# zachramsey/pm-rl

Measured on AMD Instinct MI355X. Metric: env-steps/sec (whole node) at 65k envs x 30 assets; reward MAE vs CPU ref, higher is better.
Workload: dtype f64

## Files before the change

pm-rl_amd/csrc/step_relay.h:

```cpp
#pragma once
#include "env_step.h"
#include "scalar_vec.h"

namespace pmenv_dev {

struct RelayParams {
    uint32_t scal;
    uint32_t epoch;
    uint64_t* w;
    uint64_t* list;
    uint32_t* done;
    uint32_t spin;
    uint32_t rot;
    uint32_t grid;
    const int32_t* kp_in;
    int32_t* kp_out;
    const float* halo_in;
    float* halo_out;
    uint32_t* seq;
    int32_t* kp;
    float* halo;
    uint32_t B;
    uint32_t halo_stride;
    const float* obs;
    uint32_t par;
};
enum { kSeqD = 0, kSeqE = 1, kSeqV = 2, kSeqC = 3, kSeqEC = 4, kSeqHobs = 6 };

struct RelayCtx {
    uint32_t epoch;
    const int32_t* kp_in;
    int32_t* kp_out;
    const float* halo_in;
    float* halo_out;
};
template <bool SEQ>
__device__ __forceinline__ RelayCtx relay_ctx(const RelayParams& r) {
    RelayCtx c{r.epoch, r.kp_in, r.kp_out, r.halo_in, r.halo_out};
    if constexpr (SEQ) {
        const uint32_t par = __builtin_amdgcn_readfirstlane(r.seq[kSeqC]);
        c.epoch = __builtin_amdgcn_readfirstlane(r.seq[kSeqEC]);
        c.kp_in = r.kp + (size_t)par * r.B;
        c.kp_out = r.kp + (size_t)(par ^ 1u) * r.B;
        c.halo_in = r.halo + (size_t)par * r.halo_stride;
        c.halo_out = r.halo + (size_t)(par ^ 1u) * r.halo_stride;
    }
    return c;
}

struct KArgs {
    StepParams p;
    RelayParams r;
    uint32_t qtot;
};
__device__ __forceinline__ KArgs kargs() {
    typedef __attribute__((address_space(4))) const uint32_t KWord;
    KWord* ka = (KWord*)__builtin_amdgcn_kernarg_segment_ptr();
    asm volatile("" : "+s"(ka));
    uint32_t w[sizeof(KArgs) / 4];
#pragma unroll
    for (size_t i = 0; i < sizeof(KArgs) / 4; ++i) w[i] = ka[i];
    KArgs k;
    __builtin_memcpy(&k, w, sizeof(KArgs));
    return k;
}

constexpr uint32_t kStampSlots = 16, kStampMaxWg = 40960;
static __device__ uint64_t* g_relay_stamps;
template <bool ST, bool DRAIN = false>
__device__ __forceinline__ uint64_t relay_clock(uint32_t dep) {
    uint64_t t = 0;
    if constexpr (ST) {
        if constexpr (DRAIN)
            asm volatile("s_waitcnt vmcnt(0)\n\ts_memrealtime %0\n\ts_waitcnt lgkmcnt(0)" : "=s"(t) : "v"(dep) : "memory");
        else
            asm volatile("s_memrealtime %0\n\ts_waitcnt lgkmcnt(0)" : "=s"(t) : "v"(dep) : "memory");
    }
    return t;
}
template <bool ST, int K>
__device__ __forceinline__ void relay_stamps_put(uint32_t bid, uint32_t epoch, const uint64_t (&ts)[K]) {
    if constexpr (ST) {
        uint64_t* s = g_relay_stamps;
        if (s && threadIdx.x == 0 && bid < kStampMaxWg) {
#pragma unroll
            for (int k = 0; k < K; ++k) s[((size_t)(epoch % kStampSlots) * kStampMaxWg + bid) * 8 + k] = ts[k];
        }
    }
}

__device__ __forceinline__ void relay_put(uint64_t* w, uint32_t epoch, uint32_t bits) {
    __hip_atomic_store(w, ((uint64_t)epoch << 32) | bits, __ATOMIC_RELAXED, __HIP_MEMORY_SCOPE_AGENT);
}
__device__ __forceinline__ uint64_t relay_get(const uint64_t* w) {
    return __hip_atomic_load(const_cast<uint64_t*>(w), __ATOMIC_RELAXED, __HIP_MEMORY_SCOPE_AGENT);
}

__device__ __forceinline__ uint32_t relay_list_read(const RelayParams& r, uint32_t epoch) {
    __atomic_signal_fence(__ATOMIC_SEQ_CST);
    __builtin_amdgcn_s_waitcnt(0);
    __atomic_signal_fence(__ATOMIC_SEQ_CST);
    const uint64_t lw = relay_get(r.list);
    return (uint32_t)(lw >> 32) == epoch ? (uint32_t)lw : 0u;
}

template <int BLOCK, int KL, int KA, bool ST = false>
__device__ __forceinline__ uint32_t relay_scalar(const StepParams& p, const RelayParams& r, int s, uint32_t epoch,
                                                 int32_t* kp_out, uint64_t t_entry = 0) {
    uint64_t ts[3] = {t_entry, 0, 0};
    constexpr int EPW = 64 / KL, EPB = (BLOCK / 64) * EPW;
    const int lane = threadIdx.x & 63;
    const int b = s * EPB + (int)(threadIdx.x >> 6) * EPW + lane / KL;
    const int j = lane % KL;
    const int N = p.N;
    const bool env_ok = b < p.B;
    uint32_t listed;
    if constexpr (KA == 0) {
        const ScalarIn in = scalar_load<KL>(p, b, lane);
        const ScalarMid m = scalar_core<KL>(p, b, lane, in);
        if (env_ok && j < N) relay_put(r.w + (size_t)b * N + j, epoch, __float_as_uint(m.wp));
        if (env_ok && j == 0) kp_out[b] = m.k + 1;
        listed = relay_list_read(r, epoch);
        ts[1] = relay_clock<ST>(listed);
        scalar_tail<KL>(p, b, lane, in, m);
    } else {
        const VecIn<KA> in = vec_load<KL, KA, true>(p, b, lane);
        const VecMid<KA> m = vec_core<KL, KA, true>(p, b, lane, in);
#pragma unroll
        for (int e = 0; e < KA; ++e) {
            const int n = j + e * KL;
            if (env_ok && n < N) relay_put(r.w + (size_t)b * N + n, epoch, __float_as_uint(m.wp[e]));
        }
        if (env_ok && j == 0) kp_out[b] = in.k + 1;
        listed = relay_list_read(r, epoch);
        ts[1] = relay_clock<ST>(listed);
        vec_tail<KL, KA, true>(p, b, lane, in, m);
    }
    ts[2] = relay_clock<ST, true>(0);
    relay_stamps_put<ST>((uint32_t)s, epoch, ts);
    return listed;
}

template <int BLOCK, int V, int POL, bool OUT, bool ADOPT, bool ST = false>
__device__ __forceinline__ bool relay_tile(const StepParams& p, const RelayParams& r, uint32_t qtot, uint32_t spin, uint32_t t,
                                           uint32_t epoch, const int32_t* kp_in, const float* halo_in,
                                           float* halo_out, f4* sh4, f4* sh_bar, float* sh_wp, int32_t* sh_kc,
                                           int32_t* sh_ok, uint64_t t_entry = 0) {
    uint64_t ts[6] = {t_entry, 0, 0, 0, 0, 0};
    constexpr int kAux = POL == 1 ? 2 : 0;
    constexpr int CPW = BLOCK * V, F = 5;
    const int tid = threadIdx.x, lane = tid & 63, wave = tid >> 6;
    const uint32_t c0 = t * CPW;
    const uint32_t nblk = min((uint32_t)CPW, qtot - c0);
    const auto rs = make_rsrc(p.obs + (size_t)c0 * 4, nblk * 16u);
    f4 own[V];
#pragma unroll
    for (int v = 0; v < V; ++v) own[v] = buf_load4<kAux>(rs, (uint32_t)(64 * V * wave + 64 * v + lane) * 16u);
    const uint32_t ntiles = (qtot + CPW - 1) / CPW;
    const uint32_t nh = t + 1 < ntiles ? min(2u, qtot - c0 - nblk) : 0u;
    const float* hsrc = OUT ? p.obs + (size_t)(c0 + nblk) * 4 : halo_in + (size_t)t * 8;
    const f4 hal = buf_load4<0>(make_rsrc(hsrc, nh * 16u), tid < 2 ? (uint32_t)tid * 16u : 0xFFFFFFF0u);
    __builtin_amdgcn_sched_barrier(0);
    const int N = p.N, W = p.W, WF = W * F;
    const uint32_t per4 = (uint32_t)(N * WF) >> 2;
    const uint32_t b_lo = fdiv(c0, p.div_units);
    const uint32_t g_lo = b_lo * (uint32_t)N + fdiv(4u * (c0 - b_lo * per4), p.div_wf);
    const uint32_t ql = c0 + nblk - 1u;
    const uint32_t b_hi = fdiv(ql, p.div_units);
    const uint32_t g_hi = b_hi * (uint32_t)N + fdiv(4u * (ql - b_hi * per4) + 3u, p.div_wf);
    const bool mine = (uint32_t)tid <= g_hi - g_lo;
    const uint32_t g = g_lo + (mine ? (uint32_t)tid : 0u);
    const uint32_t b = g / (uint32_t)N, n = g - b * (uint32_t)N;
    const float* barb = env_bar(p, (int)b);
    const float nanv = __int_as_float(0x7fc00000);
    f4 xb = f4{nanv, nanv, nanv, nanv};
    int32_t kc = 0;
    uint64_t ww = 0;
    if (barb) xb = *reinterpret_cast<const f4*>(barb + (size_t)n * 4);
    kc = kp_in[b];
    ww = relay_get(r.w + g);
    bool ready = !mine || (uint32_t)(ww >> 32) == epoch;
    ts[1] = relay_clock<ST>((uint32_t)ww);
    for (uint32_t polls = 0; !ADOPT && !__all(ready) && polls < spin; ++polls) {
        __builtin_amdgcn_s_sleep(2);
        if (!ready) {
            ww = relay_get(r.w + g);
            ready = (uint32_t)(ww >> 32) == epoch;
        }
    }
    const bool wave_ok = __all(ready);
    ts[2] = relay_clock<ST>((uint32_t)ww);
    if (mine) {
        sh_bar[tid] = xb;
        sh_wp[tid] = __uint_as_float((uint32_t)ww);
        sh_kc[tid] = kc;
    }
#pragma unroll
    for (int v = 0; v < V; ++v) sh4[64 * V * wave + 64 * v + lane] = own[v];
    if (tid < 2) sh4[CPW + tid] = hal;
    if (lane == 0) sh_ok[wave] = wave_ok ? 1 : 0;
    __syncthreads();
    ts[3] = relay_clock<ST>(0);
    if constexpr (ADOPT) {
        bool tile_ok = true;
#pragma unroll
        for (int w = 0; w < BLOCK / 64; ++w) tile_ok = tile_ok && sh_ok[w] != 0;
        if (!tile_ok) return false;
        if (tid == 0)
            sh_ok[BLOCK / 64] = __hip_atomic_exchange(r.done + t, epoch, __ATOMIC_RELAXED, __HIP_MEMORY_SCOPE_AGENT) != epoch;
        __syncthreads();
        if (!sh_ok[BLOCK / 64]) return true;
    }
    const auto rd = OUT ? make_rsrc(p.obs_out + (size_t)c0 * 4, nblk * 16u) : rs;
    const bool first_out = !OUT && t > 0;
    bool ok = true;
#pragma unroll
    for (int v = 0; v < V; ++v) {
        const int j = 64 * V * wave + 64 * v + lane;
        const uint32_t q = min(c0 + (uint32_t)j, qtot - 1u);
        const uint32_t bq = fdiv(q, p.div_units);
        const uint32_t j0 = 4u * (q - bq * per4);
        const uint32_t row = fdiv(j0, p.div_wf);
        const int kk = (int)(j0 - row * (uint32_t)WF);
        const int i = (int)(bq * (uint32_t)N + row - g_lo);
        const f4 n1 = sh4[j + 1], n2 = sh4[j + 2];
        const float sh[4] = {n1.y, n1.z, n1.w, n2.x};
        const float un[4] = {own[v].x, own[v].y, own[v].z, own[v].w};
        f4 o = compose2(p, kk, sh_kc[i], un, sh, [&](f4& x, float& xwp) {
            x = sh_bar[i];
            xwp = sh_wp[i];
        });
        if (!ADOPT && v == 0) {
            int32_t okv = 1;
#pragma unroll
            for (int w = 0; w < BLOCK / 64; ++w) okv &= sh_ok[w];
            ok = __builtin_amdgcn_readfirstlane(okv) != 0;
        }
        buf_store4<kAux>(rd, ok ? (uint32_t)j * 16u : 0x80000000u, o);
        if (ok && first_out && j < 2) reinterpret_cast<f4*>(halo_out)[2 * (t - 1) + j] = o;
    }
    ts[4] = relay_clock<ST>(0);
    ts[5] = relay_clock<ST, true>(0);
    relay_stamps_put<ST>(r.scal + t, epoch, ts);
    return ok;
}

template <int BLOCK, int V, int POL, bool OUT, bool SEQ>
__device__ __forceinline__ void relay_adopt(f4* sh4, f4* sh_bar, float* sh_wp, int32_t* sh_kc, int32_t* sh_ok,
                                            uint32_t listed) {
    constexpr int kB = BLOCK / 64 + 1;
    const int wave = threadIdx.x >> 6;
    if ((threadIdx.x & 63) == 0) sh_ok[wave] = (int32_t)__builtin_amdgcn_readfirstlane(listed);
    __syncthreads();
    uint32_t n = 0;
#pragma unroll
    for (int w = 0; w < BLOCK / 64; ++w) n = max(n, (uint32_t)sh_ok[w]);
    if (n == 0) return;
    const KArgs ka = kargs();
    const RelayCtx c = relay_ctx<SEQ>(ka.r);
    for (uint32_t i = 0; i < n; ++i) {
        __syncthreads();
        if (threadIdx.x == 0) {
            const uint64_t e = relay_get(ka.r.list + 1 + i);
            int32_t t = (uint32_t)(e >> 32) == c.epoch ? (int32_t)(uint32_t)e : -1;
            if (t >= 0 && __hip_atomic_load(ka.r.done + t, __ATOMIC_RELAXED, __HIP_MEMORY_SCOPE_AGENT) == c.epoch)
                t = -1;
            sh_ok[kB] = t;
        }
        __syncthreads();
        const int32_t t = __builtin_amdgcn_readfirstlane(sh_ok[kB]);
        if (t >= 0)
            (void)relay_tile<BLOCK, V, POL, OUT, true>(ka.p, ka.r, ka.qtot, 0u, (uint32_t)t, c.epoch, c.kp_in, c.halo_in,
                                                       c.halo_out, sh4, sh_bar, sh_wp, sh_kc, sh_ok);
    }
}

template <int BLOCK, int V, int POL, bool OUT, bool SEQ>
__device__ __forceinline__ void relay_defer(uint32_t t, f4* sh4, f4* sh_bar, float* sh_wp, int32_t* sh_kc,
                                            int32_t* sh_ok) {
    const KArgs ka = kargs();
    const RelayCtx c = relay_ctx<SEQ>(ka.r);
    if (threadIdx.x == 0) {
        uint64_t lw = relay_get(ka.r.list), nw;
        do {
            nw = (uint32_t)(lw >> 32) == c.epoch ? lw + 1 : ((uint64_t)c.epoch << 32) | 1u;
        } while (!__hip_atomic_compare_exchange_strong(ka.r.list, &lw, nw, __ATOMIC_RELAXED, __ATOMIC_RELAXED,
                                                        __HIP_MEMORY_SCOPE_AGENT));
        const uint32_t slot = (uint32_t)(lw >> 32) == c.epoch ? (uint32_t)lw : 0u;
        relay_put(ka.r.list + 1 + slot, c.epoch, t);
        __atomic_signal_fence(__ATOMIC_SEQ_CST);
        __builtin_amdgcn_s_waitcnt(0);
        __atomic_signal_fence(__ATOMIC_SEQ_CST);
    }
    __syncthreads();
    (void)relay_tile<BLOCK, V, POL, OUT, true>(ka.p, ka.r, ka.qtot, 0u, t, c.epoch, c.kp_in, c.halo_in, c.halo_out, sh4,
                                               sh_bar, sh_wp, sh_kc, sh_ok);
}

template <int BLOCK, int V, int POL, bool OUT, int KL, int KA, int OCC = 1, bool SEQ = false, int ANY = 0>
__global__ __launch_bounds__(BLOCK) __attribute__((amdgpu_waves_per_eu(OCC))) void step_relay_kernel(
    StepParams p, RelayParams r, uint32_t qtot) {
    __shared__ f4 sh4[BLOCK * V + 2];
    __shared__ f4 sh_bar[BLOCK];
    __shared__ float sh_wp[BLOCK];
    __shared__ int32_t sh_kc[BLOCK];
    __shared__ int32_t sh_ok[BLOCK / 64 + 2];
    const RelayCtx c = relay_ctx<SEQ>(r);
    if constexpr (SEQ) {
        if (blockIdx.x == 0 && threadIdx.x == 0) {
            const uint64_t hobs = OUT ? 0ull : (uint64_t)(uintptr_t)r.obs;
            r.seq[kSeqD] = (uint32_t)((c.kp_in - r.kp) / r.B) ^ 1u;
            r.seq[kSeqE] = c.epoch;
            r.seq[kSeqV] = 1u;
            r.seq[kSeqHobs] = (uint32_t)hobs;
            r.seq[kSeqHobs + 1] = (uint32_t)(hobs >> 32);
        }
    }
    constexpr bool kSt = ANY == 2;
    const uint64_t t_entry = relay_clock<kSt>(0);
    uint32_t bid = blockIdx.x;
    if constexpr (ANY == 1) {
        bid += r.rot;
        if (bid >= r.grid) bid -= r.grid;
    }
    if (bid < r.scal) {
        const uint32_t listed = relay_scalar<BLOCK, KL, KA, kSt>(p, r, (int)bid, c.epoch, c.kp_out, t_entry);
        relay_adopt<BLOCK, V, POL, OUT, SEQ>(sh4, sh_bar, sh_wp, sh_kc, sh_ok, listed);
    } else if (!relay_tile<BLOCK, V, POL, OUT, false, kSt>(p, r, qtot, ANY == 1 ? r.spin : kRelaySpin, bid - r.scal, c.epoch,
                                                           c.kp_in, c.halo_in, c.halo_out, sh4, sh_bar, sh_wp, sh_kc,
                                                           sh_ok, t_entry)) {
        relay_defer<BLOCK, V, POL, OUT, SEQ>(bid - r.scal, sh4, sh_bar, sh_wp, sh_kc, sh_ok);
    }
}

static __global__ __launch_bounds__(256) void relay_prime_kernel(StepParams p, RelayParams r, int prime_kp, int seq) {
    uint32_t d = r.par;
    bool kp = prime_kp != 0, halo = p.halo != nullptr;
    if (seq) {
        d = __builtin_amdgcn_readfirstlane(r.seq[kSeqD]);
        const uint32_t e = __builtin_amdgcn_readfirstlane(r.seq[kSeqE]);
        const uint32_t v = __builtin_amdgcn_readfirstlane(r.seq[kSeqV]);
        const uint64_t hobs = (uint64_t)__builtin_amdgcn_readfirstlane(r.seq[kSeqHobs]) |
                              ((uint64_t)__builtin_amdgcn_readfirstlane(r.seq[kSeqHobs + 1]) << 32);
        kp = v == 0;
        halo = halo && (v == 0 || hobs != (uint64_t)(uintptr_t)p.obs);
        if (blockIdx.x == 0 && threadIdx.x == 0) {
            r.seq[kSeqC] = d;
            r.seq[kSeqEC] = e + 1u == 0u ? 1u : e + 1u;
        }
    }
    if (halo) {
        p.halo += (size_t)d * r.halo_stride;
        copy_halo(p);
    }
    if (kp) {
        int32_t* kpd = r.kp + (size_t)d * r.B;
        for (int b = blockIdx.x * blockDim.x + threadIdx.x; b < p.B; b += gridDim.x * blockDim.x) kpd[b] = p.k[b];
    }
}

}
```

Measured before the change: 103.8 million.

## Patch new bar rows into shared image and shift uniformly in relay compose

Adds a tile-wide vote that records whether every row shifts or every row is a full-storage ring. When the tile is uniform, each owning thread writes its new bar and weight directly into the shared observation image, and the output becomes a plain four-float shift, with weight slots optionally taken from the unshifted data. This replaces the per-element index divisions and compose2 branching with simple shared-memory reads. Mixed tiles fall back to the old compose path, now with unroll disabled. The cost is an extra barrier-phase patch step and more code paths that must stay bit-exact.

Result: no change. 103.8 million (-0.0%).

```diff
diff --git a/pm-rl_amd/csrc/relay_patch.h b/pm-rl_amd/csrc/relay_patch.h
--- /dev/null
+++ b/pm-rl_amd/csrc/relay_patch.h
@@ -0,0 +1,61 @@
+#pragma once
+
+#include <stdint.h>
+
+#if defined(__HIPCC__)
+#define PMENV_HD __host__ __device__ __forceinline__
+#else
+#define PMENV_HD inline
+#endif
+
+namespace pmenv_dev {
+
+constexpr int kRelayF = 5;
+constexpr int kRelayHaloFloats = 8;
+
+enum { kVoteOk = 1, kVoteShift = 2, kVoteFull = 4 };
+
+PMENV_HD int relay_image_floats(int cpw) { return 4 * cpw + kRelayHaloFloats; }
+
+PMENV_HD bool relay_row_shifts(bool storage_ring, int32_t k, int W) { return !(storage_ring && k >= W - 1); }
+
+PMENV_HD int32_t relay_vote(bool wave_ok, bool any_shift, bool any_full) {
+    return (wave_ok ? kVoteOk : 0) | (any_shift ? kVoteShift : 0) | (any_full ? kVoteFull : 0);
+}
+PMENV_HD int32_t relay_vote_fold(int32_t all_and, int32_t all_or) {
+    return (all_and & kVoteOk) | (all_or & (kVoteShift | kVoteFull));
+}
+PMENV_HD bool relay_vote_ok(int32_t tile_vote) { return (tile_vote & kVoteOk) != 0; }
+PMENV_HD bool relay_vote_plain(int32_t tile_vote) {
+    return (tile_vote & (kVoteShift | kVoteFull)) != (kVoteShift | kVoteFull);
+}
+PMENV_HD bool relay_vote_full(int32_t tile_vote) { return (tile_vote & (kVoteShift | kVoteFull)) == kVoteFull; }
+
+PMENV_HD int relay_base0(uint32_t chunk_in_env, uint32_t row_lo, int WF) {
+    return (int)(row_lo * (uint32_t)WF) - (int)(4u * chunk_in_env);
+}
+
+PMENV_HD bool relay_in_image(int pos, int image_floats) { return (uint32_t)pos < (uint32_t)image_floats; }
+
+template <typename Put>
+PMENV_HD void relay_patch_row(int i, int base0, int WF, int image_floats, bool shifts, int slot, Put put) {
+    const int row_end = base0 + (i + 1) * WF;
+    if (relay_in_image(row_end, image_floats)) put(row_end, 0);
+    if (relay_in_image(row_end + 1, image_floats)) put(row_end + 1, 1);
+    if (relay_in_image(row_end + 2, image_floats)) put(row_end + 2, 2);
+    if (relay_in_image(row_end + 3, image_floats)) put(row_end + 3, 3);
+    const int wpos = shifts ? row_end + (kRelayF - 1) : row_end - WF + kRelayF * slot + (kRelayF - 1);
+    if (relay_in_image(wpos, image_floats)) put(wpos, kRelayF - 1);
+}
+
+PMENV_HD int relay_f0(uint32_t q) {
+    const uint32_t r = q % (uint32_t)kRelayF;
+    return r ? kRelayF - (int)r : 0;
+}
+PMENV_HD int relay_f0_step(int f0, int steps) {
+    const int f = f0 + steps % kRelayF;
+    return f >= kRelayF ? f - kRelayF : f;
+}
+PMENV_HD bool relay_is_weight(int f0, int e) { return f0 + e == kRelayF - 1 || f0 + e == 2 * kRelayF - 1; }
+
+}
diff --git a/pm-rl_amd/csrc/step_relay.h b/pm-rl_amd/csrc/step_relay.h
--- a/pm-rl_amd/csrc/step_relay.h
+++ b/pm-rl_amd/csrc/step_relay.h
@@ -1,5 +1,8 @@
 #pragma once
+#include <type_traits>
+
 #include "env_step.h"
+#include "relay_patch.h"
 #include "scalar_vec.h"
 
 namespace pmenv_dev {
@@ -190,54 +193,91 @@
     }
     const bool wave_ok = __all(ready);
     ts[2] = relay_clock<ST>((uint32_t)ww);
+    const bool shifts = relay_row_shifts(p.ring_mode == PMENV_RING_STORAGE, kc, W);
+    const int32_t wave_vote = relay_vote(wave_ok, __any(mine && shifts) != 0, __any(mine && !shifts) != 0);
+    const float wp = __uint_as_float((uint32_t)ww);
     if (mine) {
         sh_bar[tid] = xb;
-        sh_wp[tid] = __uint_as_float((uint32_t)ww);
+        sh_wp[tid] = wp;
         sh_kc[tid] = kc;
     }
 #pragma unroll
     for (int v = 0; v < V; ++v) sh4[64 * V * wave + 64 * v + lane] = own[v];
     if (tid < 2) sh4[CPW + tid] = hal;
-    if (lane == 0) sh_ok[wave] = wave_ok ? 1 : 0;
+    if (lane == 0) sh_ok[wave] = wave_vote;
+    __syncthreads();
+    int32_t v_and = kVoteOk, v_or = 0;
+#pragma unroll
+    for (int w = 0; w < BLOCK / 64; ++w) {
+        const int32_t x = sh_ok[w];
+        v_and &= x;
+        v_or |= x;
+    }
+    const int32_t vote = __builtin_amdgcn_readfirstlane(relay_vote_fold(v_and, v_or));
+    if constexpr (ADOPT) {
+        if (!relay_vote_ok(vote)) return false;
+        if (tid == 0)
+            sh_ok[BLOCK / 64] = __hip_atomic_exchange(r.done + t, epoch, __ATOMIC_RELAXED, __HIP_MEMORY_SCOPE_AGENT) != epoch;
+    }
+    const bool plain = relay_vote_plain(vote), full = relay_vote_full(vote);
+    if (plain && mine) {
+        const uint32_t cq = c0 - b_lo * per4;
+        const int slot = (int)((uint32_t)(1 + kc) - fdiv((uint32_t)(1 + kc), p.div_w) * (uint32_t)W);
+        float* img = reinterpret_cast<float*>(sh4);
+        relay_patch_row(tid, relay_base0(cq, g_lo - b_lo * (uint32_t)N, WF), WF, relay_image_floats(CPW), shifts, slot,
+                        [&](int pos, int c) { img[pos] = c == 0 ? xb.x : c == 1 ? xb.y : c == 2 ? xb.z : c == 3 ? xb.w : wp; });
+    }
     __syncthreads();
     ts[3] = relay_clock<ST>(0);
     if constexpr (ADOPT) {
-        bool tile_ok = true;
-#pragma unroll
-        for (int w = 0; w < BLOCK / 64; ++w) tile_ok = tile_ok && sh_ok[w] != 0;
-        if (!tile_ok) return false;
-        if (tid == 0)
-            sh_ok[BLOCK / 64] = __hip_atomic_exchange(r.done + t, epoch, __ATOMIC_RELAXED, __HIP_MEMORY_SCOPE_AGENT) != epoch;
-        __syncthreads();
         if (!sh_ok[BLOCK / 64]) return true;
     }
     const auto rd = OUT ? make_rsrc(p.obs_out + (size_t)c0 * 4, nblk * 16u) : rs;
     const bool first_out = !OUT && t > 0;
-    bool ok = true;
-#pragma unroll
-    for (int v = 0; v < V; ++v) {
-        const int j = 64 * V * wave + 64 * v + lane;
-        const uint32_t q = min(c0 + (uint32_t)j, qtot - 1u);
-        const uint32_t bq = fdiv(q, p.div_units);
-        const uint32_t j0 = 4u * (q - bq * per4);
-        const uint32_t row = fdiv(j0, p.div_wf);
-        const int kk = (int)(j0 - row * (uint32_t)WF);
-        const int i = (int)(bq * (uint32_t)N + row - g_lo);
-        const f4 n1 = sh4[j + 1], n2 = sh4[j + 2];
-        const float sh[4] = {n1.y, n1.z, n1.w, n2.x};
-        const float un[4] = {own[v].x, own[v].y, own[v].z, own[v].w};
-        f4 o = compose2(p, kk, sh_kc[i], un, sh, [&](f4& x, float& xwp) {
-            x = sh_bar[i];
-            xwp = sh_wp[i];
-        });
-        if (!ADOPT && v == 0) {
-            int32_t okv = 1;
-#pragma unroll
-            for (int w = 0; w < BLOCK / 64; ++w) okv &= sh_ok[w];
-            ok = __builtin_amdgcn_readfirstlane(okv) != 0;
-        }
+    const bool ok = ADOPT || relay_vote_ok(vote);
+    auto put = [&](int j, const f4& o) {
         buf_store4<kAux>(rd, ok ? (uint32_t)j * 16u : 0x80000000u, o);
         if (ok && first_out && j < 2) reinterpret_cast<f4*>(halo_out)[2 * (t - 1) + j] = o;
+    };
+    if (plain) {
+        const int f0 = relay_f0(c0 + (uint32_t)(64 * V * wave + lane));
+        auto shift_all = [&](auto own_w) {
+#pragma unroll
+            for (int v = 0; v < V; ++v) {
+                const int j = 64 * V * wave + 64 * v + lane;
+                const f4 n1 = sh4[j + 1], n2 = sh4[j + 2];
+                f4 o = f4{n1.y, n1.z, n1.w, n2.x};
+                if constexpr (decltype(own_w)::value) {
+                    const f4 n0 = sh4[j];
+                    const int f = relay_f0_step(f0, v);
+                    o.x = relay_is_weight(f, 0) ? n0.x : o.x;
+                    o.y = relay_is_weight(f, 1) ? n0.y : o.y;
+                    o.z = relay_is_weight(f, 2) ? n0.z : o.z;
+                    o.w = relay_is_weight(f, 3) ? n0.w : o.w;
+                }
+                put(j, o);
+            }
+        };
+        if (full) shift_all(std::true_type{});
+        else shift_all(std::false_type{});
+    } else {
+#pragma unroll 1
+        for (int v = 0; v < V; ++v) {
+            const int j = 64 * V * wave + 64 * v + lane;
+            const uint32_t q = min(c0 + (uint32_t)j, qtot - 1u);
+            const uint32_t bq = fdiv(q, p.div_units);
+            const uint32_t j0 = 4u * (q - bq * per4);
+            const uint32_t row = fdiv(j0, p.div_wf);
+            const int kk = (int)(j0 - row * (uint32_t)WF);
+            const int i = (int)(bq * (uint32_t)N + row - g_lo);
+            const f4 n0 = sh4[j], n1 = sh4[j + 1], n2 = sh4[j + 2];
+            const float sh[4] = {n1.y, n1.z, n1.w, n2.x};
+            const float un[4] = {n0.x, n0.y, n0.z, n0.w};
+            put(j, compose2(p, kk, sh_kc[i], un, sh, [&](f4& x, float& xwp) {
+                x = sh_bar[i];
+                xwp = sh_wp[i];
+            }));
+        }
     }
     ts[4] = relay_clock<ST>(0);
     ts[5] = relay_clock<ST, true>(0);
```
